# xu-ji/IIC

Measured on AMD Instinct MI355X. Metric: paired-images/sec, STL10 96x96 ClusterNet5g+IID_loss, higher is better.
Workload: dtype bf16; 1 GPU; STL10 96x96 ClusterNet5g IID+ (cluster_sobel.py train step), batch 660 pairs/GPU, 5 sub-heads, k=70, bf16 MFMA convs / fp32 stem+heads+loss, fused HIP Adam; global_batch_pairs=660, input=96x96x1 grey -> sobel 2ch, parallelism=dp1, streams=2, launch=hip-graph replay: 6 linear graph segments, the two views on two streams

## Files before the change

iic_amd/csrc/conv_igemm_bd.hip:

```cpp
#include "common.h"
#include "conv_tile.h"
#include "../../include/iic_hip.h"

__device__ __forceinline__ void bd_bload(u32x4& d, const unsigned char* p) {
  asm volatile("global_load_dwordx4 %0, %1, off" : "=v"(d) : "v"(p) : "memory");
}
template <int N>
__device__ __forceinline__ void bd_bwait(u32x4& d) {
  asm volatile("s_waitcnt vmcnt(%1)" : "+v"(d) : "i"(N) : "memory");
}

struct bd_blk {
  int bw, bh, nbx, nby;
  int PW, npix, mul;
};

#define BD_BM 256
#define BD_BN 128
#define BD_THREADS 256
#define BD_PROF_SLOTS 16
#ifndef BD_STORE_UB
#define BD_STORE_UB 8
#endif

// ... 293 lines not shown
      if (lane < 32) {
        const int col = wn * 64 + ns * 32 + lane;
        s_red[(wm * 2 + 0) * BNT + col] = s;
        s_red[(wm * 2 + 1) * BNT + col] = ss;
      }
    }
  }
  __syncthreads();
  if (stats && tid < BNT && !(ABL & 64)) {
    const int stripe = blockIdx.x % IIC_STAT_STRIPES;
    float a0 = 0.f, a1 = 0.f;
#pragma unroll
    for (int q = 0; q < NWM; ++q) {
      a0 += s_red[(q * 2 + 0) * BNT + tid];
      a1 += s_red[(q * 2 + 1) * BNT + tid];
    }
    iic_stat_add(stats, stripe, g.Cout, n0 + tid, 0, a0);
    iic_stat_add(stats, stripe, g.Cout, n0 + tid, 1, a1);
  }
#pragma unroll
  for (int ms = 0; ms < MS; ++ms)
#pragma unroll
    for (int ns = 0; ns < 2; ++ns)
#pragma unroll
      for (int r = 0; r < 16; ++r) {
        const int row = wm * WR + ms * 32 + mfma32_row(r, lane);
        const int col = wn * 64 + ns * 32 + l31;
        sC[row * CLD + col] = f32_to_bf16(acc[ms][ns][r]);
      }
  __syncthreads();
  if (PROF) t_stamp[4] = __builtin_readcyclecounter();
  TileRed tr;
  if (RED) tile_red_zero(tr);
  if (!(ABL & 32))
    igemm_store_tile<BNT, BM, BD_THREADS, 8, RED, (BM == 256 ? BD_STORE_UB : 4)>(sC, s_pout, out, res_grad, res_act, accumulate,
                                                                 g.Cout, n0, tid, red_y, red_coef, red_y2, &tr);
  if (RED)
    igemm_red_finish<BNT, BD_THREADS, RED>(tr, reinterpret_cast<float*>(smem_raw), red_stats, red_stats2,
                                             g.Cout, n0, tid);
  if (PROF && prof && tid == 0) {
    unsigned long long* q = prof + (long)blockIdx.x * BD_PROF_SLOTS;
    const unsigned long long t_end = __builtin_readcyclecounter();
    q[0] = t_stamp[0]; q[1] = t_stamp[1]; q[2] = t_stamp[2]; q[3] = t_stamp[3]; q[4] = t_stamp[4];
    q[5] = t_end; q[6] = t_bsum; q[7] = (unsigned long long)t_nb;
    q[8] = (unsigned long long)__builtin_amdgcn_s_getreg((32 - 1) << 11 | 0 << 6 | 4)
           | ((unsigned long long)__builtin_amdgcn_s_getreg((4 - 1) << 11 | 0 << 6 | 20) << 32);
    q[9] = (unsigned long long)tix;
    q[10] = __builtin_amdgcn_s_memrealtime();
  }
}

template <bool GATHER, int ABL, int MS, int RED, int WN = 2>
__global__ __launch_bounds__(BD_THREADS, ((MS == 4 || WN == 1) ? 2 : 3)) void conv_igemm_bd_kernel(
    const iic_conv_geom g, const bf16_t* __restrict__ in, const unsigned char* __restrict__ wfrag,
    bf16_t* __restrict__ out, float* __restrict__ stats, const bf16_t* __restrict__ res_grad,
    const bf16_t* __restrict__ res_act, int accumulate, int num_mtiles, int lds_a_bytes,
    const bf16_t* __restrict__ red_y, const float* __restrict__ red_coef,
    const bf16_t* __restrict__ red_y2, float* __restrict__ red_stats, float* __restrict__ red_stats2,
    unsigned long long* __restrict__ prof, const bd_blk B) {
  bd_tile<GATHER, ABL, MS, RED, WN>(g, in, wfrag, out, stats, res_grad, res_act, accumulate, lds_a_bytes, red_y,
                                    red_coef, red_y2, red_stats, red_stats2, prof, (int)blockIdx.x,
                                    num_mtiles * (g.Cout / (WN * 64)), B);
}

__global__ void weight_prep_frag_kernel(const float* __restrict__ w, bf16_t* __restrict__ o, int Co,
                                        int Ci, int T, int mode) {
  const int Nn = mode ? Ci : Co, Kk = mode ? Co : Ci;
  const int n32 = Nn >> 5, nchunks = Kk >> 6;
  const long total = (long)T * Co * Ci;
  for (long i = (long)blockIdx.x * blockDim.x + threadIdx.x; i < total;
       i += (long)gridDim.x * blockDim.x) {
    const int e = (int)(i & 7), lane = (int)((i >> 3) & 63), ks = (int)((i >> 9) & 3);
    long r = i >> 11;
    const int j = (int)(r % n32);
    r /= n32;
    const int kc = (int)(r % nchunks), t = (int)(r / nchunks);
    const int n = j * 32 + (lane & 31), k = kc * 64 + ks * 16 + (lane >> 5) * 8 + e;
    const int co = mode ? k : n, ci = mode ? n : k;
    o[i] = f32_to_bf16(w[((long)co * Ci + ci) * T + t]);
  }
}

int iic_p64_supported(const iic_conv_geom* g);
int iic_p64_launch(const iic_conv_geom* g, const void* in, const void* wfrag, void* out, float* stats,
                   const void* res_grad, const void* res_act, int accumulate, const void* red_y,
                   const float* red_coef, const void* red_y2, float* red_stats, float* red_stats2,
                   void* stream);
int iic_pw_supported(const iic_conv_geom* g);
int iic_pw_launch(const iic_conv_geom* g, const void* in, const void* wfrag, void* out, float* stats,
                  const void* res_grad, const void* res_act, int accumulate, const void* red_y,
                  const float* red_coef, const void* red_y2, float* red_stats, float* red_stats2, void* stream);
IIC_SWITCH(g_p64_enabled, 1, iic_debug_enable_p64)
IIC_SWITCH(g_p64_red, 0, iic_debug_p64_red)

extern "C" {

#ifdef IIC_DEBUG_HOOKS
static unsigned long long* g_bd_prof = nullptr;
IIC_HOOK void iic_debug_bd_prof(void* buf) { g_bd_prof = (unsigned long long*)buf; }
IIC_HOOK int iic_debug_bd_prof_slots(void) { return BD_PROF_SLOTS; }
#else
static constexpr unsigned long long* g_bd_prof = nullptr;
#endif

static long bd_lds_a(const iic_conv_geom* g, int ms, int wn = 2) {
  const long bm = ms * 32 * (4 / wn);
  const long npix = g->ntaps == 1 ? bm : (bm >= 192 ? g->NP256 : g->NP);
  long a = (npix * 128 + 1023) & ~1023L;
  long c = bm * (wn * 64 + 8) * 2;
  long m = a > c ? a : c;
  return (m + 15) & ~15L;
}

static long bd_key_bytes(const iic_conv_geom* g, int ms, int wn = 2) {
  const int jskip = (g->ntaps > 1 && g->sx == 1 && ((g->in_Wp - g->MX) & 1) == 0) ? g->in_Wp - g->MX : 0;
  return jskip != 0 ? (((long)(ms * 32 * (4 / wn) >= 192 ? g->NP256 : g->NP) + 15) & ~15L) : 0;
}
static long bd_lds_total(const iic_conv_geom* g, int ms, int wn = 2) {
  return bd_lds_a(g, ms, wn) + 2L * ms * 32 * (4 / wn) * 4 + 4L * BD_BN * 4 + bd_key_bytes(g, ms, wn);
}
IIC_SWITCH(g_bd_w1, 1, iic_debug_bd_w1)
static bool bd_w1_ok(const iic_conv_geom* g) {
  return g_bd_w1 && g->Cout % 64 == 0 && g->Cout % BD_BN != 0 && g->ntaps > 1 && g->NP256 > 0 &&
         bd_lds_total(g, 2, 1) <= 160 * 1024;
}
IIC_SWITCH(g_bd_ms, 0, iic_debug_bd_ms)
static int bd_pick_ms(const iic_conv_geom* g) {
  const bool ok4 = (g->ntaps == 1 || g->NP256 > 0) && bd_lds_total(g, 4) <= 160 * 1024;
  const bool ok2 = (g->ntaps == 1 || g->NP > 0) && bd_lds_total(g, 2) <= 160 * 1024;
  if (g_bd_ms == 4) return ok4 ? 4 : (ok2 ? 2 : 0);
  if (g_bd_ms == 2) return ok2 ? 2 : (ok4 ? 4 : 0);
  if (ok4 && ok2 && g->ntaps > 1) {
    const long M = igemm_rows_host(g);
    if (((M + 255) / 256) * (g->Cout / BD_BN) * 2 <= 512) return 2;
  }
  return ok4 ? 4 : (ok2 ? 2 : 0);
}

static int bd_block_config(const iic_conv_geom* g, bd_blk* B, int wn);
int iic_conv_igemm_frag_supported(const iic_conv_geom* g) {
  if (!g) return 0;
  if (g_p64_enabled && iic_p64_supported(g)) return 1;
  if (g->Cin % 64 != 0 || g->ntaps < 1 || g->ntaps > IIC_MAX_TAPS) return 0;
  bd_blk B;
  if (g->Cout % BD_BN != 0) return (bd_w1_ok(g) || (g->Cout % 64 == 0 && bd_block_config(g, &B, 1))) ? 1 : 0;
  return bd_pick_ms(g) != 0 || bd_block_config(g, &B, 2) != 0;
}

int iic_conv_igemm_frag_red(const iic_conv_geom* g, const void* in, const void* wfrag, void* out,
                            float* stats, const void* res_grad, const void* res_act, int accumulate,
                            const void* red_y, const float* red_coef, const void* red_y2,
                            float* red_stats, float* red_stats2, void* stream);

IIC_SWITCH(g_bd_blk, 1, iic_debug_bd_blk)
static int bd_block_config(const iic_conv_geom* g, bd_blk* B, int wn) {
  B->bw = 0;
  if (!g_bd_blk || g->ntaps < 2 || g->Cout % (wn * 64) != 0 || g->Cin % 64 != 0) return 0;
  if (g->sy != 1 || g->sx != 1 || g->ty != 1 || g->tx != 1 || g->MY < 32 || g->MX < 32 || g->NP256 <= 0) return 0;
  int mix = 0, miy = 0;
  for (int t = 0; t < g->ntaps; ++t) {
    const int iy = g->tap_off[t] / g->in_Wp, ix = g->tap_off[t] % g->in_Wp;
    if (ix > 8 || iy > 8) return 0;
    mix = ix > mix ? ix : mix;
    miy = iy > miy ? iy : miy;
  }
  if (mix & 1) return 0;
  double best = -1.0;
  int best_bw = 0;
  long best_tiles = 0;
  for (int bw = 8; bw <= 64 && bw <= g->MX; ++bw) {
    const int bh = BD_BM / bw;
    if (bh < 2 || bh > g->MY) continue;
    const long tiles = (long)((g->MX + bw - 1) / bw) * ((g->MY + bh - 1) / bh);
    const long npix = (long)(bw + mix) * (bh + miy);
    const long a = (npix * 128 + 1023) & ~1023L;
    const long c = (long)BD_BM * (wn * 64 + 8) * 2;
    const long tot = (a > c ? a : c) + 2L * BD_BM * 4 + 4L * BD_BN * 4 + ((npix + 15) & ~15L);
    if (tot > 80 * 1024 || npix >= 65536 / (bw + mix)) continue;
    const double cost = (double)tiles * (1.0 + 0.5 * (double)npix * 128.0 / 32768.0);
    if (best < 0 || cost < best) { best = cost; best_bw = bw; best_tiles = tiles; }
  }
  if (best < 0) return 0;
  const int bw = best_bw, bh = BD_BM / bw;
  if ((double)g->MY * g->MX < 0.88 * (double)BD_BM * (double)best_tiles) return 0;
  const int npix = (bw + mix) * (bh + miy);
  if (g_bd_blk != 2 && !(bd_lds_total(g, wn == 2 ? 4 : 2, wn) > 80 * 1024 || npix * 10 < g->NP256 * 7)) return 0;
  B->bw = bw; B->bh = bh;
  B->nbx = (g->MX + bw - 1) / bw; B->nby = (g->MY + bh - 1) / bh;
  B->PW = bw + mix; B->npix = npix; B->mul = (65536 + B->PW - 1) / B->PW;
  return 1;
}

int iic_conv_igemm_red_supported(const iic_conv_geom* g) {
  if (!g || !iic_conv_igemm_frag_supported(g)) return 0;
  if (g_p64_enabled && iic_p64_supported(g)) return g_p64_red;
  return g->ntaps > 1;
}

int iic_conv_igemm_frag(const iic_conv_geom* g, const void* in, const void* wfrag, void* out,
                        float* stats, const void* res_grad, const void* res_act, int accumulate,
                        void* stream) {
  return iic_conv_igemm_frag_red(g, in, wfrag, out, stats, res_grad, res_act, accumulate, nullptr, nullptr,
                                 nullptr, nullptr, nullptr, stream);
}

int iic_conv_igemm_frag_red(const iic_conv_geom* g, const void* in, const void* wfrag, void* out,
                            float* stats, const void* res_grad, const void* res_act, int accumulate,
                            const void* red_y, const float* red_coef, const void* red_y2,
                            float* red_stats, float* red_stats2, void* stream) {
  if (!g || !in || !wfrag || !out) return IIC_ERR_ARG;
  if ((red_y == nullptr) != (red_stats == nullptr) || (red_y2 == nullptr) != (red_stats2 == nullptr) ||
      (red_y2 && !red_y) || (red_coef && !red_y))
    return IIC_ERR_ARG;
  const int red = red_y ? (red_y2 ? 2 : 1) : 0;
  if (!(accumulate & IIC_ACC_PREMASK) && (res_grad == nullptr) != (res_act == nullptr)) return IIC_ERR_ARG;
  if (!iic_conv_igemm_frag_supported(g)) return IIC_ERR_UNSUPPORTED;
  if (g_p64_enabled && iic_p64_supported(g)) {
    if (red && !g_p64_red) return IIC_ERR_UNSUPPORTED;
    return iic_p64_launch(g, in, wfrag, out, stats, res_grad, res_act, accumulate, red_y, red_coef, red_y2,
                          red_stats, red_stats2, stream);
  }
  if (iic_debug_get_ablate() == 0 && g_bd_ms == 0 && iic_pw_supported(g))
    return iic_pw_launch(g, in, wfrag, out, stats, res_grad, res_act, accumulate, red_y, red_coef, red_y2, red_stats,
                         red_stats2, stream);
  const long M = igemm_rows_host(g);
  if (M <= 0) return IIC_ERR_ARG;
  if (M >= (1L << 31) || (long)g->N * g->in_Hp * g->in_Wp >= (1L << 31)) return IIC_ERR_UNSUPPORTED;
  if (g->Cout % BD_BN != 0) {
    bd_blk B1 = {0, 0, 0, 0, 0, 0, 0};
    const bool blocked1 = bd_block_config(g, &B1, 1) != 0;
    const int mt1 = blocked1 ? g->N * B1.nbx * B1.nby : (int)((M + 255) / 256);
    const int grid1 = mt1 * (g->Cout / 64);
    int la1 = (int)bd_lds_a(g, 2, 1);
    long lds1 = bd_lds_total(g, 2, 1);
    if (blocked1) {
      const long a = ((long)B1.npix * 128 + 1023) & ~1023L, c = (long)BD_BM * (64 + 8) * 2;
      la1 = (int)(((a > c ? a : c) + 15) & ~15L);
      lds1 = la1 + 2L * BD_BM * 4 + 4L * BD_BN * 4 + ((B1.npix + 15) & ~15L);
    }
    hipStream_t s1 = (hipStream_t)stream;
#define BD_LAUNCH_W1(RD_)                                                                              \
  do {                                                                                                 \
    static bool attr = false;                                                                          \
    if (!attr) {                                                                                       \
      (void)hipFuncSetAttribute(                                                                       \
          reinterpret_cast<const void*>(&conv_igemm_bd_kernel<false, 0, 2, RD_, 1>),          \
          hipFuncAttributeMaxDynamicSharedMemorySize, 160 * 1024);                                     \
      attr = true;                                                                                     \
    }                                                                                                  \
    hipLaunchKernelGGL((conv_igemm_bd_kernel<false, 0, 2, RD_, 1>), dim3(grid1),              \
                       dim3(BD_THREADS), lds1, s1, *g, (const bf16_t*)in, (const unsigned char*)wfrag, \
                       (bf16_t*)out, stats, (const bf16_t*)res_grad, (const bf16_t*)res_act,           \
                       accumulate, mt1, la1, (const bf16_t*)red_y, red_coef, (const bf16_t*)red_y2,    \
                       red_stats, red_stats2, (unsigned long long*)nullptr, B1);                       \
  } while (0)
    if (red == 0) BD_LAUNCH_W1(0); else if (red == 1) BD_LAUNCH_W1(1); else BD_LAUNCH_W1(2);
    return iic_launch_status();
  }
  bd_blk BB = {0, 0, 0, 0, 0, 0, 0};
  const bool blocked = iic_debug_get_ablate() == 0 && bd_block_config(g, &BB, 2) != 0;
  const int ms = blocked ? 4 : bd_pick_ms(g);
  if (ms == 0) return IIC_ERR_UNSUPPORTED;
  const int bm = ms * 64;
  const int mt = blocked ? g->N * BB.nbx * BB.nby : (int)((M + bm - 1) / bm);
  const int nt = g->Cout / BD_BN;
  const int grid = mt * nt;
  int la = (int)bd_lds_a(g, ms);
  long lds = bd_lds_total(g, ms);
  if (blocked) {
    const long a = ((long)BB.npix * 128 + 1023) & ~1023L, c = (long)BD_BM * (BD_BN + 8) * 2;
    la = (int)(((a > c ? a : c) + 15) & ~15L);
    lds = la + 2L * BD_BM * 4 + 4L * BD_BN * 4 + ((BB.npix + 15) & ~15L);
  }
  hipStream_t s = (hipStream_t)stream;
#define BD_LAUNCH4(GA_, AB_, MS_, RD_)                                                            \
  do {                                                                                           \
    static bool attr = false;                                                                    \
    if (!attr) {                                                                                 \
      (void)hipFuncSetAttribute(                                                                 \
          reinterpret_cast<const void*>(&conv_igemm_bd_kernel<GA_, AB_, MS_, RD_>),              \
          hipFuncAttributeMaxDynamicSharedMemorySize, 160 * 1024);                               \
      attr = true;                                                                               \
    }                                                                                            \
    hipLaunchKernelGGL((conv_igemm_bd_kernel<GA_, AB_, MS_, RD_>), dim3(grid),                   \
                       dim3(BD_THREADS), lds, s, *g, (const bf16_t*)in,                          \
                       (const unsigned char*)wfrag, (bf16_t*)out, stats, (const bf16_t*)res_grad, \
                       (const bf16_t*)res_act, accumulate, mt, la, (const bf16_t*)red_y,         \
                       red_coef, (const bf16_t*)red_y2, red_stats, red_stats2, g_bd_prof, BB);   \
  } while (0)
#define BD_LAUNCH3(GA_, AB_, MS_)                                                                 \
  do {                                                                                           \
    if ((AB_ != 0 && AB_ != 128 && AB_ != 256) || GA_ || red == 0) {                             \
      if (red != 0) return IIC_ERR_UNSUPPORTED;                                                  \
      BD_LAUNCH4(GA_, AB_, MS_, 0);                                                              \
    } else if (red == 1) BD_LAUNCH4(false, (AB_ == 128 || AB_ == 256 ? AB_ : 0), MS_, 1);        \
    else BD_LAUNCH4(false, (AB_ == 128 || AB_ == 256 ? AB_ : 0), MS_, 2);                        \
  } while (0)
#define BD_LAUNCH(GA_, AB_)                                                                       \
  do {                                                                                           \
    if (ms == 4) BD_LAUNCH3(GA_, AB_, 4); else BD_LAUNCH3(GA_, AB_, 2);                          \
  } while (0)
  if (g->ntaps == 1) BD_LAUNCH(true, 0);
  else switch (iic_debug_get_ablate()) {
// ... 86 lines not shown
```

iic_amd/csrc/conv_igemm_p64.hip:

```cpp
#include "common.h"
#include "conv_tile.h"
#include "../../include/iic_hip.h"

#define P64_BM 256
#define P64_BN 64
#define P64_THREADS 512
#define P64_NT 9
#define P64_CLD P64_BN
#define P64_SC_BYTES(BM_) ((BM_) * P64_CLD * 2)
#define P64_NTAB 4
#define P64_TAB_BYTES(BM_) (P64_NTAB * (BM_) * (4 + 2))

struct P64Walk {
  int n, y, x;
};
__device__ __forceinline__ void p64_walk_init(P64Walk& w, const iic_conv_geom& g, int m) {
  const int plane = g.MY * g.MX;
  w.n = m / plane;
  const int r = m - w.n * plane;
  w.y = r / g.MX;
  w.x = r - w.y * g.MX;
}
__device__ __forceinline__ void p64_walk_advance(P64Walk& w, const iic_conv_geom& g, int d_y, int d_x) {
  w.x += d_x;
  w.y += d_y;
  if (w.x >= g.MX) { w.x -= g.MX; ++w.y; }
  while (w.y >= g.MY) { w.y -= g.MY; ++w.n; }
}
__device__ __forceinline__ void p64_walk_pixels(const P64Walk& w, const iic_conv_geom& g, int& pin,
                                                int& pout) {
  const bool valid = w.n < g.N;
  const int n = valid ? w.n : g.N - 1, y = valid ? w.y : g.MY - 1, x = valid ? w.x : g.MX - 1;
  pin = (n * g.in_Hp + y * g.sy + g.oy) * g.in_Wp + x * g.sx + g.ox;
  pout = valid ? (n * g.out_Hp + y * g.ty + g.py) * g.out_Wp + x * g.tx + g.px : -1;
}

template <int ABL, int RED>
__global__ __launch_bounds__(512) void conv_igemm_p64_kernel(
    const iic_conv_geom g, const bf16_t* __restrict__ in, const unsigned char* __restrict__ wfrag,
    bf16_t* __restrict__ out, float* __restrict__ stats, const bf16_t* __restrict__ res_grad,
    const bf16_t* __restrict__ res_act, int accumulate, int num_tiles, int pb_bytes, int max_tap_off,
    const bf16_t* __restrict__ red_y, const float* __restrict__ red_coef,
    const bf16_t* __restrict__ red_y2, float* __restrict__ red_stats, float* __restrict__ red_stats2,
    unsigned long long* __restrict__ prof) {
  constexpr bool PROF = (ABL & 8) != 0;
  constexpr int NW = 8, BM = P64_BM;
  constexpr int NWM = BM / 64;
  constexpr int SC_BYTES = BM * P64_CLD * 2, TAB_ROWS = P64_NTAB * BM;
  unsigned long long ph[6] = {0, 0, 0, 0, 0, 0}, t_a = 0, t_b = 0, t_loop = 0;
  extern __shared__ __attribute__((aligned(16))) unsigned char smem_raw[];
  unsigned char* const sP0 = smem_raw;
  unsigned char* const sP1 = smem_raw + pb_bytes;
  bf16_t* const sC = reinterpret_cast<bf16_t*>(smem_raw + 2 * pb_bytes);
  int* const s_pout = reinterpret_cast<int*>(smem_raw + 2 * pb_bytes + SC_BYTES);
  unsigned short* const s_prow = reinterpret_cast<unsigned short*>(s_pout + TAB_ROWS);
  float* const s_red = reinterpret_cast<float*>(sC);

  constexpr int NTH = NW * 64;
  constexpr int NCO = 1;
  const int tid = threadIdx.x, lane = tid & 63;
  const int wave = __builtin_amdgcn_readfirstlane(tid >> 6);
  const int wm = wave >> 1, wn = wave & 1;
  const int l31 = lane & 31, g5 = lane >> 5;
  const int M = g.N * g.MY * g.MX;
  const int in_pixels = g.N * g.in_Hp * g.in_Wp;

  const int G = gridDim.x;
  const int wl = xcd_tile_index(blockIdx.x, G);
  const int t0 = (int)(((long)wl * num_tiles) / G), t1 = (int)(((long)(wl + 1) * num_tiles) / G);
  if (t0 >= t1) return;

  const int v_tapoff = g.tap_off[lane & (IIC_MAX_TAPS - 1)];
  const int d_y = BM / g.MX, d_x = BM - d_y * g.MX;

  P64Walk wr, w0, w255;
  p64_walk_init(wr, g, t0 * BM + (tid & (BM - 1)));
  p64_walk_init(w0, g, t0 * BM);
  p64_walk_init(w255, g, t0 * BM + BM - 1);
  int plo_q[3], nblk_q[3];
  auto tabulate = [&](int t) {
    int pin, pout, p0, p255, dummy;
    p64_walk_pixels(w0, g, p0, dummy);
    p64_walk_pixels(w255, g, p255, dummy);
    p0 = __builtin_amdgcn_readfirstlane(p0);
    p255 = __builtin_amdgcn_readfirstlane(p255);
    if (tid < BM) {
      p64_walk_pixels(wr, g, pin, pout);
      s_pout[(t & (P64_NTAB - 1)) * BM + tid] = pout;
      s_prow[(t & (P64_NTAB - 1)) * BM + tid] = (unsigned short)(pin - p0);
    }
    p64_walk_advance(wr, g, d_y, d_x);
    p64_walk_advance(w0, g, d_y, d_x);
    p64_walk_advance(w255, g, d_y, d_x);
    plo_q[0] = plo_q[1];
    nblk_q[0] = nblk_q[1];
    plo_q[1] = plo_q[2];
    nblk_q[1] = nblk_q[2];
    plo_q[2] = p0;
    nblk_q[2] = ((p255 + max_tap_off - p0 + 1) * 128 + 1023) >> 10;
  };
  auto dma_issue = [&](unsigned char* dst, int plo, int nblk) {
    for (int blk = wave; blk < nblk; blk += NW) {
      const int q = blk * 64 + lane;
      const int r = q >> 3;
      const int ls = (q & 7) ^ ((r >> 1) & 7);
      int p = plo + r;
      p = p < in_pixels ? p : in_pixels - 1;
      __builtin_amdgcn_global_load_lds(
          (const __attribute__((address_space(1))) void*)(in + ((long)p * 64 + ls * 8)),
          (__attribute__((address_space(3))) void*)(dst + blk * 1024), 16, 0, 0);
    }
  };

  tabulate(t0);
  tabulate(t0 + 1);
  dma_issue(sP0, plo_q[1], nblk_q[1]);
  u32x4 Bw[P64_NT][NCO][4];
#pragma unroll
  for (int tap = 0; tap < P64_NT; ++tap)
#pragma unroll
    for (int c = 0; c < NCO; ++c) {
      const unsigned char* p = wfrag + ((long)g.tap_w[tap] * 2 + wn + c) * 4096 + lane * 16;
#pragma unroll
      for (int ks = 0; ks < 4; ++ks) Bw[tap][c][ks] = *reinterpret_cast<const u32x4*>(p + ks * 1024);
    }
  f32x2 st_s[NCO], st_ss[NCO];
#pragma unroll
  for (int c = 0; c < NCO; ++c) {
    st_s[c] = f32x2{0.f, 0.f};
    st_ss[c] = f32x2{0.f, 0.f};
  }
  TileRed tr;
  if (RED) tile_red_zero(tr);

  if (PROF) t_loop = __builtin_readcyclecounter();
  for (int t = t0; t < t1; ++t) {
    const int par = (t - t0) & 1;
    unsigned char* const sP = par ? sP1 : sP0;
    if (PROF) t_a = __builtin_readcyclecounter();
    asm volatile("s_waitcnt vmcnt(0)" ::: "memory");
    __syncthreads();
    if (PROF) { t_b = __builtin_readcyclecounter(); ph[0] += t_b - t_a; t_a = t_b; }
    const bool spread = RED == 0 && !res_grad && !res_act && !accumulate;
    if (t > t0 && !(ABL & 2) && !spread)
      igemm_store_tile<P64_BN, BM, NTH, 0, RED, (RED ? 1 : 4)>(sC, s_pout + ((t - 1) & (P64_NTAB - 1)) * BM,
                                                            out, res_grad, res_act, accumulate, P64_BN, 0, tid,
                                                            red_y, red_coef, red_y2, &tr);
    if (PROF) { t_b = __builtin_readcyclecounter(); ph[1] += t_b - t_a; t_a = t_b; }
    if (t + 1 < t1 && !(ABL & 1)) dma_issue(par ? sP0 : sP1, plo_q[2], nblk_q[2]);
    tabulate(t + 2);
    if (PROF) { t_b = __builtin_readcyclecounter(); ph[2] += t_b - t_a; t_a = t_b; }
    int R0[2];
#pragma unroll
    for (int ms = 0; ms < 2; ++ms)
      R0[ms] = s_prow[(t & (P64_NTAB - 1)) * BM + wm * 64 + ms * 32 + l31];
    f32x16 acc[2][NCO];
    constexpr int NTAPS = (ABL & 4) ? 1 : P64_NT;
    auto load_a = [&](int tap, bf16x8 (&a)[2][4]) {
      const int toff = __builtin_amdgcn_readlane(v_tapoff, tap);
#pragma unroll
      for (int ms = 0; ms < 2; ++ms) {
        const int R = R0[ms] + toff;
        const int key = (R >> 1) & 7;
        const int base = R * 128 + (((g5 ^ key) & 1) << 4);
        const int kk = (key >> 1) << 5;
#pragma unroll
        for (int ks = 0; ks < 4; ++ks)
          a[ms][ks] = *reinterpret_cast<const bf16x8*>(sP + base + ((ks << 5) ^ kk));
      }
    };
#pragma unroll
    for (int tap = 0; tap < NTAPS; ++tap) {
      bf16x8 a[2][4];
      load_a(tap, a);
      if (spread && t > t0 && !(ABL & 2)) {
        constexpr int SIT = BM * 8 / NTH;
        constexpr int PER = (SIT + P64_NT - 2) / (P64_NT - 1);
#pragma unroll
        for (int q = 0; q < PER; ++q) {
          const int it = (tap - 1) * PER + q;
          if (tap >= 1 && it < SIT) {
            const int idx = tid + it * NTH;
            const int row = idx >> 3, ch = idx & 7;
            const int po = s_pout[((t - 1) & (P64_NTAB - 1)) * BM + row];
            if (po >= 0)
              *reinterpret_cast<uint4*>(out + (long)po * P64_BN + ch * 8) =
                  *reinterpret_cast<const uint4*>(sC + row * P64_CLD + ch * 8);
          }
        }
      }
#pragma unroll
      for (int ks = 0; ks < 4; ++ks)
#pragma unroll
        for (int c = 0; c < NCO; ++c) {
          const bf16x8 b = __builtin_bit_cast(bf16x8, Bw[tap][c][ks]);
          if (tap == 0 && ks == 0) {
            const f32x16 z = {0.f, 0.f, 0.f, 0.f, 0.f, 0.f, 0.f, 0.f, 0.f, 0.f, 0.f, 0.f, 0.f, 0.f, 0.f, 0.f};
            acc[0][c] = __builtin_amdgcn_mfma_f32_32x32x16_bf16(a[0][ks], b, z, 0, 0, 0);
            acc[1][c] = __builtin_amdgcn_mfma_f32_32x32x16_bf16(a[1][ks], b, z, 0, 0, 0);
          } else {
            acc[0][c] = __builtin_amdgcn_mfma_f32_32x32x16_bf16(a[0][ks], b, acc[0][c], 0, 0, 0);
            acc[1][c] = __builtin_amdgcn_mfma_f32_32x32x16_bf16(a[1][ks], b, acc[1][c], 0, 0, 0);
          }
        }
    }
    if (stats) {
      if ((t + 1) * BM > M) {
#pragma unroll
        for (int ms = 0; ms < 2; ++ms)
#pragma unroll
          for (int r = 0; r < 16; ++r)
            if (t * BM + wm * 64 + ms * 32 + mfma32_row(r, lane) >= M) {
#pragma unroll
              for (int c = 0; c < NCO; ++c) acc[ms][c][r] = 0.f;
            }
      }
#pragma unroll
      for (int c = 0; c < NCO; ++c)
#pragma unroll
        for (int ms = 0; ms < 2; ++ms)
#pragma unroll
          for (int r = 0; r < 16; r += 2) {
            const f32x2 v = {acc[ms][c][r], acc[ms][c][r + 1]};
            st_s[c] += v;
            st_ss[c] += v * v;
          }
    }
    if (PROF) { t_b = __builtin_readcyclecounter(); ph[3] += t_b - t_a; t_a = t_b; }
    asm volatile("s_waitcnt lgkmcnt(0)" ::: "memory");
    __builtin_amdgcn_s_barrier();
    if (PROF) { t_b = __builtin_readcyclecounter(); ph[4] += t_b - t_a; t_a = t_b; }
#pragma unroll
    for (int c = 0; c < NCO; ++c)
#pragma unroll
      for (int ms = 0; ms < 2; ++ms)
#pragma unroll
        for (int r = 0; r < 16; ++r)
          sC[(wm * 64 + ms * 32 + mfma32_row(r, lane)) * P64_CLD + (wn + c) * 32 + l31] = f32_to_bf16(acc[ms][c][r]);
    if (PROF) { t_b = __builtin_readcyclecounter(); ph[5] += t_b - t_a; }
  }
  if (PROF && prof && tid == 0) {
    unsigned long long* q = prof + (long)blockIdx.x * 8;
#pragma unroll
    for (int i = 0; i < 6; ++i) q[i] = ph[i];
    q[6] = (unsigned long long)(t1 - t0);
    q[7] = __builtin_readcyclecounter() - t_loop;
  }

  __syncthreads();
  if (!(ABL & 2))
    igemm_store_tile<P64_BN, BM, NTH, 0, RED, (RED ? 1 : 4)>(sC, s_pout + ((t1 - 1) & (P64_NTAB - 1)) * BM, out,
                                                          res_grad, res_act, accumulate, P64_BN, 0, tid,
                                                          red_y, red_coef, red_y2, &tr);
  if (RED)
    igemm_red_finish<P64_BN, NTH, RED>(tr, reinterpret_cast<float*>(sC), red_stats, red_stats2, P64_BN,
                                               0, tid);
  if (stats) {
    __syncthreads();
#pragma unroll
    for (int c = 0; c < NCO; ++c) {
      float s1 = st_s[c][0] + st_s[c][1], s2 = st_ss[c][0] + st_ss[c][1];
      s1 += __shfl_xor(s1, 32, 64);
      s2 += __shfl_xor(s2, 32, 64);
      if (lane < 32) {
        s_red[(wm * 2 + 0) * P64_BN + (wn + c) * 32 + lane] = s1;
        s_red[(wm * 2 + 1) * P64_BN + (wn + c) * 32 + lane] = s2;
      }
    }
    __syncthreads();
    if (tid < P64_BN) {
      float a0 = 0.f, a1 = 0.f;
#pragma unroll
      for (int q = 0; q < NWM; ++q) {
        a0 += s_red[(q * 2 + 0) * P64_BN + tid];
        a1 += s_red[(q * 2 + 1) * P64_BN + tid];
      }
      const int stripe = blockIdx.x % IIC_STAT_STRIPES;
      iic_stat_add(stats, stripe, P64_BN, tid, 0, a0);
      iic_stat_add(stats, stripe, P64_BN, tid, 1, a1);
    }
  }
}

#ifdef IIC_DEBUG_HOOKS
static unsigned long long* g_p64_prof = nullptr;
IIC_HOOK void iic_debug_p64_prof(void* buf) { g_p64_prof = (unsigned long long*)buf; }
#else
static constexpr unsigned long long* g_p64_prof = nullptr;
#endif
IIC_SWITCH(g_p64_grid, 0, iic_debug_p64_grid)

static int p64_num_cus() {
  if (g_p64_grid > 0) return g_p64_grid;
  static int n = 0;
  if (n == 0) {
    int dev = 0, v = 0;
    if (hipGetDevice(&dev) == hipSuccess &&
        hipDeviceGetAttribute(&v, hipDeviceAttributeMultiprocessorCount, dev) == hipSuccess && v > 0)
      n = v;
    else
      n = 256;
  }
  return n;
}

static long p64_pb_bytes(const iic_conv_geom* g, int bm = P64_BM) {
  return (((long)(bm == 128 ? g->NP : g->NP256) * 128) + 1023) & ~1023L;
}

int iic_p64_supported(const iic_conv_geom* g) {
  if (g->Cin != 64 || g->Cout != 64 || g->ntaps != P64_NT || g->NP256 <= 0 || g->NP256 > 65535) return 0;
  if (!igemm_dense_host(g)) return 0;
  return 2 * p64_pb_bytes(g) + P64_SC_BYTES(P64_BM) + P64_TAB_BYTES(P64_BM) <= 160 * 1024;
}

int iic_p64_launch(const iic_conv_geom* g, const void* in, const void* wfrag, void* out, float* stats,
                   const void* res_grad, const void* res_act, int accumulate, const void* red_y,
                   const float* red_coef, const void* red_y2, float* red_stats, float* red_stats2,
                   void* stream) {
  const int red = red_y ? (red_y2 ? 2 : 1) : 0;
  const long M = (long)g->N * g->MY * g->MX;
  if (M <= 0) return IIC_ERR_ARG;
  if (M >= (1L << 31) - P64_BM || (long)g->N * g->in_Hp * g->in_Wp >= (1L << 31)) return IIC_ERR_UNSUPPORTED;
  const int bm = P64_BM;
  const int nt = (int)((M + bm - 1) / bm);
  const int pb = (int)p64_pb_bytes(g, bm);
  const long lds = 2L * pb + P64_SC_BYTES(bm) + P64_TAB_BYTES(bm);
  int mto = 0;
  for (int i = 0; i < g->ntaps; ++i) mto = g->tap_off[i] > mto ? g->tap_off[i] : mto;
  const int ncu = p64_num_cus();
  const int grid = nt < ncu ? nt : ncu;
#define P64_LAUNCH2(AB_, RD_)                                                                          \
  do {                                                                                                 \
    static bool attr = false;                                                                          \
    if (!attr) {                                                                                       \
      (void)hipFuncSetAttribute(reinterpret_cast<const void*>(&conv_igemm_p64_kernel<AB_, RD_>),       \
                                hipFuncAttributeMaxDynamicSharedMemorySize, 160 * 1024);               \
      attr = true;                                                                                     \
    }                                                                                                  \
    hipLaunchKernelGGL((conv_igemm_p64_kernel<AB_, RD_>), dim3(grid), dim3(512), lds,                  \
                       (hipStream_t)stream, *g, (const bf16_t*)in, (const unsigned char*)wfrag,   \
                       (bf16_t*)out, stats, (const bf16_t*)res_grad, (const bf16_t*)res_act,      \
                       accumulate, nt, pb, mto, (const bf16_t*)red_y, red_coef,                   \
                       (const bf16_t*)red_y2, red_stats, red_stats2, g_p64_prof);                 \
  } while (0)
#define P64_LAUNCH(AB_) P64_LAUNCH2(AB_, 0)
  if (red == 1) { P64_LAUNCH2(0, 1); return iic_launch_status(); }
  if (red == 2) { P64_LAUNCH2(0, 2); return iic_launch_status(); }
  switch (iic_debug_get_ablate()) {
#ifdef IIC_BD_ABLATIONS
    case 1: P64_LAUNCH(1); break;
    case 2: P64_LAUNCH(2); break;
    case 3: P64_LAUNCH(3); break;
    case 4: P64_LAUNCH(4); break;
    case 7: P64_LAUNCH(7); break;
    case 8: P64_LAUNCH(8); break;
#endif
    default: P64_LAUNCH(0); break;
  }
  return iic_launch_status();
}
```

iic_amd/csrc/conv_tile.h:

```cpp
#pragma once
#include "common.h"
#include "../../include/iic_hip.h"

__device__ __forceinline__ void igemm_row_pixels(const iic_conv_geom& g, int m, int& pin, int& pout) {
  const int plane = g.MY * g.MX;
  const int mp = g.MP > 0 ? g.MP : plane;
  int n = m / mp;
  int r = m - n * mp;
  const bool valid = n < g.N && r < plane;
  if (n >= g.N) { n = g.N - 1; r = plane - 1; }
  r = r < plane ? r : plane - 1;
  const int y = r / g.MX, x = r - y * g.MX;
  pin = (n * g.in_Hp + y * g.sy + g.oy) * g.in_Wp + x * g.sx + g.ox;
  pout = valid ? (n * g.out_Hp + y * g.ty + g.py) * g.out_Wp + x * g.tx + g.px : -1;
}
__device__ __forceinline__ int igemm_rows(const iic_conv_geom& g) {
  return g.N * (g.MP > 0 ? g.MP : g.MY * g.MX);
}
__device__ __forceinline__ bool igemm_tile_has_invalid(const iic_conv_geom& g, int m0, int bm) {
  const int plane = g.MY * g.MX;
  if (m0 + bm > igemm_rows(g)) return true;
  return g.MP > 0 && g.MP != plane && (m0 % g.MP) + bm > plane;
}
static inline long igemm_rows_host(const iic_conv_geom* g) {
// ... 74 lines not shown
      const int idx = tid + (b0 + u) * NTHREADS;
      const int row = idx / CH;
      const int po = (idx < BM * CH) ? s_pout[row] : -1;
      o[u] = po < 0 ? -1 : (long)po * Cout + n0 + ch * 8;
      if (o[u] >= 0) {
        if (add_prev) pv[u] = *reinterpret_cast<const uint4*>(out + o[u]);
        if (res_grad) gv[u] = *reinterpret_cast<const uint4*>(res_grad + o[u]);
        if (res_act) av[u] = *reinterpret_cast<const uint4*>(res_act + o[u]);
        if (RED) yv[u] = *reinterpret_cast<const uint4*>(red_y + o[u]);
        if (RED == 2) zv[u] = *reinterpret_cast<const uint4*>(red_y2 + o[u]);
      }
    }
#pragma unroll
    for (int u = 0; u < U; ++u) {
      if (o[u] < 0) continue;
      const int row = (tid + (b0 + u) * NTHREADS) / CH;
      uint4 v = *reinterpret_cast<const uint4*>(sC + row * CLD + ch * 8);
      if (any_in) {
        uint32_t vv[4] = {v.x, v.y, v.z, v.w};
        float f[8];
#pragma unroll
        for (int i = 0; i < 4; ++i) { f[2 * i] = bf16lo(vv[i]); f[2 * i + 1] = bf16hi(vv[i]); }
        if (add_prev) {
          const uint32_t oo[4] = {pv[u].x, pv[u].y, pv[u].z, pv[u].w};
#pragma unroll
          for (int i = 0; i < 4; ++i) { f[2 * i] += bf16lo(oo[i]); f[2 * i + 1] += bf16hi(oo[i]); }
        }
        if (premask) {
          if (res_grad) {
            const uint32_t gg[4] = {gv[u].x, gv[u].y, gv[u].z, gv[u].w};
#pragma unroll
            for (int i = 0; i < 4; ++i) { f[2 * i] += bf16lo(gg[i]); f[2 * i + 1] += bf16hi(gg[i]); }
          }
          if (res_act) {
            const uint32_t aa[4] = {av[u].x, av[u].y, av[u].z, av[u].w};
#pragma unroll
            for (int i = 0; i < 4; ++i) {
              if (!(bf16lo(aa[i]) > 0.f)) f[2 * i] = 0.f;
              if (!(bf16hi(aa[i]) > 0.f)) f[2 * i + 1] = 0.f;
            }
          }
        } else if (res_grad) {
          const uint32_t gg[4] = {gv[u].x, gv[u].y, gv[u].z, gv[u].w};
          const uint32_t aa[4] = {av[u].x, av[u].y, av[u].z, av[u].w};
#pragma unroll
          for (int i = 0; i < 4; ++i) {
            if (bf16lo(aa[i]) > 0.f) f[2 * i] += bf16lo(gg[i]);
            if (bf16hi(aa[i]) > 0.f) f[2 * i + 1] += bf16hi(gg[i]);
          }
        }
        v = make_uint4(pack_bf16x2(f[0], f[1]), pack_bf16x2(f[2], f[3]), pack_bf16x2(f[4], f[5]),
                       pack_bf16x2(f[6], f[7]));
      }
      *reinterpret_cast<uint4*>(out + o[u]) = v;
      if (RED) {
        const uint32_t gq4[4] = {v.x, v.y, v.z, v.w};
        const uint32_t yy[4] = {yv[u].x, yv[u].y, yv[u].z, yv[u].w};
        float gq[8], yq[8];
#pragma unroll
        for (int i = 0; i < 4; ++i) {
          gq[2 * i] = bf16lo(gq4[i]); gq[2 * i + 1] = bf16hi(gq4[i]);
          yq[2 * i] = bf16lo(yy[i]); yq[2 * i + 1] = bf16hi(yy[i]);
        }
        if (red_coef) {
#pragma unroll
          for (int i = 0; i < 8; ++i)
            if (!(yq[i] * msc[RED ? i : 0] + msh[RED ? i : 0] > 0.f)) gq[i] = 0.f;
        }
#pragma unroll
        for (int i = 0; i < 8; ++i) { red->s[i] += gq[i]; red->sy[i] += gq[i] * yq[i]; }
        if (RED == 2) {
          const uint32_t zz[4] = {zv[u].x, zv[u].y, zv[u].z, zv[u].w};
#pragma unroll
          for (int i = 0; i < 4; ++i) {
            red->sy2[2 * i] += gq[2 * i] * bf16lo(zz[i]);
            red->sy2[2 * i + 1] += gq[2 * i + 1] * bf16hi(zz[i]);
          }
        }
      }
    }
  }
}

template <int BN, int NTHREADS, int RED>
__device__ __forceinline__ void igemm_red_finish(TileRed& r, float* scratch, float* red_stats,
                                                 float* red_stats2, int Cout, int n0, int tid) {
  constexpr int CH = BN / 8, NW = NTHREADS / 64;
  static_assert(64 % CH == 0, "channel chunks must divide the wave");
  const int lane = tid & 63, wave = tid >> 6, ch = tid % CH;
#pragma unroll
  for (int i = 0; i < 8; ++i) {
#pragma unroll
    for (int o = CH; o < 64; o <<= 1) {
      r.s[i] += __shfl_xor(r.s[i], o, 64);
      r.sy[i] += __shfl_xor(r.sy[i], o, 64);
      if (RED == 2) r.sy2[i] += __shfl_xor(r.sy2[i], o, 64);
    }
  }
  __syncthreads();
  if (lane < CH) {
#pragma unroll
    for (int i = 0; i < 8; ++i) {
      scratch[(wave * 3 + 0) * BN + ch * 8 + i] = r.s[i];
      scratch[(wave * 3 + 1) * BN + ch * 8 + i] = r.sy[i];
      if (RED == 2) scratch[(wave * 3 + 2) * BN + ch * 8 + i] = r.sy2[i];
    }
  }
  __syncthreads();
  if (tid < BN) {
    float a0 = 0.f, a1 = 0.f, a2 = 0.f;
    for (int w = 0; w < NW; ++w) {
      a0 += scratch[(w * 3 + 0) * BN + tid];
      a1 += scratch[(w * 3 + 1) * BN + tid];
      if (RED == 2) a2 += scratch[(w * 3 + 2) * BN + tid];
    }
    const int stripe = blockIdx.x % IIC_STAT_STRIPES;
    iic_stat_add(red_stats, stripe, Cout, n0 + tid, 0, a0);
    iic_stat_add(red_stats, stripe, Cout, n0 + tid, 1, a1);
    if (RED == 2) {
      iic_stat_add(red_stats2, stripe, Cout, n0 + tid, 0, a0);
      iic_stat_add(red_stats2, stripe, Cout, n0 + tid, 1, a2);
    }
  }
}
```

Before: 18750 paired-images/sec.

## Interleave p64 conv epilogue stores with MFMA tap loop for residual/reduction paths

Adds an EPI template variant of the p64 implicit-GEMM kernel. For tiles with residual, accumulate or reduction epilogues, it splits the previous tile's store into pieces and issues their global loads and stores between the taps of the current tile's MFMA loop, instead of running a separate store phase before the compute. This is meant to hide epilogue memory latency behind the matrix math. Reduction coefficients are staged in LDS, which needs extra LDS and adds new support checks. Fused stats with red are now rejected, and red==2 keeps the non-pipelined path.

```diff
diff --git a/iic_amd/csrc/conv_igemm_bd.hip b/iic_amd/csrc/conv_igemm_bd.hip
--- a/iic_amd/csrc/conv_igemm_bd.hip
+++ b/iic_amd/csrc/conv_igemm_bd.hip
@@ -399,10 +399,11 @@
 }
 
 int iic_p64_supported(const iic_conv_geom* g);
+int iic_p64_red_supported(const iic_conv_geom* g);
 int iic_p64_launch(const iic_conv_geom* g, const void* in, const void* wfrag, void* out, float* stats,
                    const void* res_grad, const void* res_act, int accumulate, const void* red_y,
                    const float* red_coef, const void* red_y2, float* red_stats, float* red_stats2,
-                   void* stream);
+                   int pipelined, void* stream);
 int iic_pw_supported(const iic_conv_geom* g);
 int iic_pw_launch(const iic_conv_geom* g, const void* in, const void* wfrag, void* out, float* stats,
                   const void* res_grad, const void* res_act, int accumulate, const void* red_y,
@@ -510,7 +511,7 @@
 
 int iic_conv_igemm_red_supported(const iic_conv_geom* g) {
   if (!g || !iic_conv_igemm_frag_supported(g)) return 0;
-  if (g_p64_enabled && iic_p64_supported(g)) return g_p64_red;
+  if (g_p64_enabled && iic_p64_supported(g)) return g_p64_red && iic_p64_red_supported(g);
   return g->ntaps > 1;
 }
 
@@ -533,9 +534,9 @@
   if (!(accumulate & IIC_ACC_PREMASK) && (res_grad == nullptr) != (res_act == nullptr)) return IIC_ERR_ARG;
   if (!iic_conv_igemm_frag_supported(g)) return IIC_ERR_UNSUPPORTED;
   if (g_p64_enabled && iic_p64_supported(g)) {
-    if (red && !g_p64_red) return IIC_ERR_UNSUPPORTED;
+    if (red && !(g_p64_red && iic_p64_red_supported(g))) return IIC_ERR_UNSUPPORTED;
     return iic_p64_launch(g, in, wfrag, out, stats, res_grad, res_act, accumulate, red_y, red_coef, red_y2,
-                          red_stats, red_stats2, stream);
+                          red_stats, red_stats2, g_p64_red, stream);
   }
   if (iic_debug_get_ablate() == 0 && g_bd_ms == 0 && iic_pw_supported(g))
     return iic_pw_launch(g, in, wfrag, out, stats, res_grad, res_act, accumulate, red_y, red_coef, red_y2, red_stats,
diff --git a/iic_amd/csrc/conv_igemm_p64.hip b/iic_amd/csrc/conv_igemm_p64.hip
--- a/iic_amd/csrc/conv_igemm_p64.hip
+++ b/iic_amd/csrc/conv_igemm_p64.hip
@@ -10,6 +10,7 @@
 #define P64_SC_BYTES(BM_) ((BM_) * P64_CLD * 2)
 #define P64_NTAB 4
 #define P64_TAB_BYTES(BM_) (P64_NTAB * (BM_) * (4 + 2))
+#define P64_COEF_BYTES (2 * P64_BN * 4)
 
 struct P64Walk {
   int n, y, x;
@@ -35,7 +36,7 @@
   pout = valid ? (n * g.out_Hp + y * g.ty + g.py) * g.out_Wp + x * g.tx + g.px : -1;
 }
 
-template <int ABL, int RED>
+template <int ABL, int RED, int EPI>
 __global__ __launch_bounds__(512) void conv_igemm_p64_kernel(
     const iic_conv_geom g, const bf16_t* __restrict__ in, const unsigned char* __restrict__ wfrag,
     bf16_t* __restrict__ out, float* __restrict__ stats, const bf16_t* __restrict__ res_grad,
@@ -55,6 +56,7 @@
   int* const s_pout = reinterpret_cast<int*>(smem_raw + 2 * pb_bytes + SC_BYTES);
   unsigned short* const s_prow = reinterpret_cast<unsigned short*>(s_pout + TAB_ROWS);
   float* const s_red = reinterpret_cast<float*>(sC);
+  float* const s_coef = reinterpret_cast<float*>(s_prow + TAB_ROWS);
 
   constexpr int NTH = NW * 64;
   constexpr int NCO = 1;
@@ -132,6 +134,8 @@
   }
   TileRed tr;
   if (RED) tile_red_zero(tr);
+  if (EPI && RED && red_coef && tid < 2 * P64_BN) s_coef[tid] = red_coef[tid];
+  const bool add_prev = accumulate & IIC_ACC_ADD, premask = accumulate & IIC_ACC_PREMASK;
 
   if (PROF) t_loop = __builtin_readcyclecounter();
   for (int t = t0; t < t1; ++t) {
@@ -142,7 +146,7 @@
     __syncthreads();
     if (PROF) { t_b = __builtin_readcyclecounter(); ph[0] += t_b - t_a; t_a = t_b; }
     const bool spread = RED == 0 && !res_grad && !res_act && !accumulate;
-    if (t > t0 && !(ABL & 2) && !spread)
+    if (!EPI && t > t0 && !(ABL & 2) && !spread)
       igemm_store_tile<P64_BN, BM, NTH, 0, RED, (RED ? 1 : 4)>(sC, s_pout + ((t - 1) & (P64_NTAB - 1)) * BM,
                                                             out, res_grad, res_act, accumulate, P64_BN, 0, tid,
                                                             red_y, red_coef, red_y2, &tr);
@@ -169,6 +173,51 @@
           a[ms][ks] = *reinterpret_cast<const bf16x8*>(sP + base + ((ks << 5) ^ kk));
       }
     };
+    if constexpr (EPI != 0) {
+      TilePiece<RED> pc;
+      int pc_po = -1;
+      const int ch = tid & 7;
+      const bool pipe = t > t0 && !(ABL & 2);
+      const int* const po_tab = s_pout + ((t - 1) & (P64_NTAB - 1)) * BM;
+#pragma unroll
+      for (int tap = 0; tap < NTAPS; ++tap) {
+        if (pipe && (tap & 1) == 0) {
+          if (tap >= 2 && pc_po >= 0) {
+            pc.o = (long)pc_po * P64_BN + ch * 8;
+            const int row = (tap / 2 - 1) * (NTH / 8) + (tid >> 3);
+            const uint4 v = *reinterpret_cast<const uint4*>(sC + row * P64_CLD + ch * 8);
+            igemm_piece_finish<RED>(pc, v, out, res_grad != nullptr, res_act != nullptr, add_prev, premask,
+                                    red_coef != nullptr, s_coef + ch * 8, s_coef + P64_BN + ch * 8, &tr);
+          }
+          if (tap < 8) {
+            pc_po = po_tab[(tap / 2) * (NTH / 8) + (tid >> 3)];
+            pc.o = (long)pc_po * P64_BN + ch * 8;
+            if (pc_po >= 0) igemm_piece_load<RED>(pc, out, res_grad, res_act, add_prev, red_y, red_y2);
+          }
+        }
+        const int toff = __builtin_amdgcn_readlane(v_tapoff, tap);
+#pragma unroll
+        for (int ms = 0; ms < 2; ++ms) {
+          const int R = R0[ms] + toff;
+          const int key = (R >> 1) & 7;
+          const int base = R * 128 + (((g5 ^ key) & 1) << 4);
+          const int kk = (key >> 1) << 5;
+          bf16x8 a[4];
+#pragma unroll
+          for (int ks = 0; ks < 4; ++ks) a[ks] = *reinterpret_cast<const bf16x8*>(sP + base + ((ks << 5) ^ kk));
+#pragma unroll
+          for (int ks = 0; ks < 4; ++ks) {
+            const bf16x8 b = __builtin_bit_cast(bf16x8, Bw[tap][0][ks]);
+            if (tap == 0 && ks == 0) {
+              const f32x16 z = {0.f, 0.f, 0.f, 0.f, 0.f, 0.f, 0.f, 0.f, 0.f, 0.f, 0.f, 0.f, 0.f, 0.f, 0.f, 0.f};
+              acc[ms][0] = __builtin_amdgcn_mfma_f32_32x32x16_bf16(a[ks], b, z, 0, 0, 0);
+            } else {
+              acc[ms][0] = __builtin_amdgcn_mfma_f32_32x32x16_bf16(a[ks], b, acc[ms][0], 0, 0, 0);
+            }
+          }
+        }
+      }
+    } else {
 #pragma unroll
     for (int tap = 0; tap < NTAPS; ++tap) {
       bf16x8 a[2][4];
@@ -204,7 +253,8 @@
           }
         }
     }
-    if (stats) {
+    }
+    if (RED == 0 && stats) {
       if ((t + 1) * BM > M) {
 #pragma unroll
         for (int ms = 0; ms < 2; ++ms)
@@ -255,7 +305,7 @@
   if (RED)
     igemm_red_finish<P64_BN, NTH, RED>(tr, reinterpret_cast<float*>(sC), red_stats, red_stats2, P64_BN,
                                                0, tid);
-  if (stats) {
+  if (RED == 0 && stats) {
     __syncthreads();
 #pragma unroll
     for (int c = 0; c < NCO; ++c) {
@@ -313,11 +363,15 @@
   if (!igemm_dense_host(g)) return 0;
   return 2 * p64_pb_bytes(g) + P64_SC_BYTES(P64_BM) + P64_TAB_BYTES(P64_BM) <= 160 * 1024;
 }
+int iic_p64_red_supported(const iic_conv_geom* g) {
+  return iic_p64_supported(g) &&
+         2 * p64_pb_bytes(g) + P64_SC_BYTES(P64_BM) + P64_TAB_BYTES(P64_BM) + P64_COEF_BYTES <= 160 * 1024;
+}
 
 int iic_p64_launch(const iic_conv_geom* g, const void* in, const void* wfrag, void* out, float* stats,
                    const void* res_grad, const void* res_act, int accumulate, const void* red_y,
                    const float* red_coef, const void* red_y2, float* red_stats, float* red_stats2,
-                   void* stream) {
+                   int pipelined, void* stream) {
   const int red = red_y ? (red_y2 ? 2 : 1) : 0;
   const long M = (long)g->N * g->MY * g->MX;
   if (M <= 0) return IIC_ERR_ARG;
@@ -325,38 +379,41 @@
   const int bm = P64_BM;
   const int nt = (int)((M + bm - 1) / bm);
   const int pb = (int)p64_pb_bytes(g, bm);
-  const long lds = 2L * pb + P64_SC_BYTES(bm) + P64_TAB_BYTES(bm);
+  const bool epi = pipelined && (red || res_grad || res_act || accumulate);
+  const long lds = 2L * pb + P64_SC_BYTES(bm) + P64_TAB_BYTES(bm) + (red ? P64_COEF_BYTES : 0);
+  if (lds > 160 * 1024) return IIC_ERR_UNSUPPORTED;
   int mto = 0;
   for (int i = 0; i < g->ntaps; ++i) mto = g->tap_off[i] > mto ? g->tap_off[i] : mto;
   const int ncu = p64_num_cus();
   const int grid = nt < ncu ? nt : ncu;
-#define P64_LAUNCH2(AB_, RD_)                                                                          \
+#define P64_LAUNCH(AB_, RD_, EP_)                                                                      \
   do {                                                                                                 \
     static bool attr = false;                                                                          \
     if (!attr) {                                                                                       \
-      (void)hipFuncSetAttribute(reinterpret_cast<const void*>(&conv_igemm_p64_kernel<AB_, RD_>),       \
+      (void)hipFuncSetAttribute(reinterpret_cast<const void*>(&conv_igemm_p64_kernel<AB_, RD_, EP_>),  \
                                 hipFuncAttributeMaxDynamicSharedMemorySize, 160 * 1024);               \
       attr = true;                                                                                     \
     }                                                                                                  \
-    hipLaunchKernelGGL((conv_igemm_p64_kernel<AB_, RD_>), dim3(grid), dim3(512), lds,                  \
-                       (hipStream_t)stream, *g, (const bf16_t*)in, (const unsigned char*)wfrag,   \
-                       (bf16_t*)out, stats, (const bf16_t*)res_grad, (const bf16_t*)res_act,      \
-                       accumulate, nt, pb, mto, (const bf16_t*)red_y, red_coef,                   \
-                       (const bf16_t*)red_y2, red_stats, red_stats2, g_p64_prof);                 \
+    hipLaunchKernelGGL((conv_igemm_p64_kernel<AB_, RD_, EP_>), dim3(grid), dim3(512), lds,             \
+                       (hipStream_t)stream, *g, (const bf16_t*)in, (const unsigned char*)wfrag,        \
+                       (bf16_t*)out, stats, (const bf16_t*)res_grad, (const bf16_t*)res_act,           \
+                       accumulate, nt, pb, mto, (const bf16_t*)red_y, red_coef,                        \
+                       (const bf16_t*)red_y2, red_stats, red_stats2, g_p64_prof);                      \
   } while (0)
-#define P64_LAUNCH(AB_) P64_LAUNCH2(AB_, 0)
-  if (red == 1) { P64_LAUNCH2(0, 1); return iic_launch_status(); }
-  if (red == 2) { P64_LAUNCH2(0, 2); return iic_launch_status(); }
+  if (red && stats) return IIC_ERR_UNSUPPORTED;
+  if (red && !pipelined) return IIC_ERR_UNSUPPORTED;
+  if (red == 1) { P64_LAUNCH(0, 1, 1); return iic_launch_status(); }
+  if (red == 2) { P64_LAUNCH(0, 2, 0); return iic_launch_status(); }
   switch (iic_debug_get_ablate()) {
 #ifdef IIC_BD_ABLATIONS
-    case 1: P64_LAUNCH(1); break;
-    case 2: P64_LAUNCH(2); break;
-    case 3: P64_LAUNCH(3); break;
-    case 4: P64_LAUNCH(4); break;
-    case 7: P64_LAUNCH(7); break;
-    case 8: P64_LAUNCH(8); break;
+    case 1: P64_LAUNCH(1, 0, 0); break;
+    case 2: P64_LAUNCH(2, 0, 0); break;
+    case 3: P64_LAUNCH(3, 0, 0); break;
+    case 4: P64_LAUNCH(4, 0, 0); break;
+    case 7: P64_LAUNCH(7, 0, 0); break;
+    case 8: if (epi) P64_LAUNCH(8, 0, 1); else P64_LAUNCH(8, 0, 0); break;
 #endif
-    default: P64_LAUNCH(0); break;
+    default: if (epi) P64_LAUNCH(0, 0, 1); else P64_LAUNCH(0, 0, 0); break;
   }
   return iic_launch_status();
 }
diff --git a/iic_amd/csrc/conv_tile.h b/iic_amd/csrc/conv_tile.h
--- a/iic_amd/csrc/conv_tile.h
+++ b/iic_amd/csrc/conv_tile.h
@@ -180,6 +180,94 @@
   }
 }
 
+template <int RED>
+struct TilePiece {
+  long o;
+  uint4 pv, gv, av, yv, zv;
+};
+
+template <int RED>
+__device__ __forceinline__ void igemm_piece_load(TilePiece<RED>& p, const bf16_t* __restrict__ out,
+                                                 const bf16_t* __restrict__ res_grad,
+                                                 const bf16_t* __restrict__ res_act, bool add_prev,
+                                                 const bf16_t* __restrict__ red_y,
+                                                 const bf16_t* __restrict__ red_y2) {
+  if (add_prev) p.pv = *reinterpret_cast<const uint4*>(out + p.o);
+  if (res_grad) p.gv = *reinterpret_cast<const uint4*>(res_grad + p.o);
+  if (res_act) p.av = *reinterpret_cast<const uint4*>(res_act + p.o);
+  if (RED) p.yv = *reinterpret_cast<const uint4*>(red_y + p.o);
+  if (RED == 2) p.zv = *reinterpret_cast<const uint4*>(red_y2 + p.o);
+}
+
+template <int RED>
+__device__ __forceinline__ void igemm_piece_finish(const TilePiece<RED>& p, uint4 v, bf16_t* __restrict__ out,
+                                                   bool has_grad, bool has_act, bool add_prev, bool premask,
+                                                   bool has_coef, const float* msc, const float* msh,
+                                                   TileRed* red) {
+  if (add_prev || has_grad || has_act) {
+    uint32_t vv[4] = {v.x, v.y, v.z, v.w};
+    float f[8];
+#pragma unroll
+    for (int i = 0; i < 4; ++i) { f[2 * i] = bf16lo(vv[i]); f[2 * i + 1] = bf16hi(vv[i]); }
+    if (add_prev) {
+      const uint32_t oo[4] = {p.pv.x, p.pv.y, p.pv.z, p.pv.w};
+#pragma unroll
+      for (int i = 0; i < 4; ++i) { f[2 * i] += bf16lo(oo[i]); f[2 * i + 1] += bf16hi(oo[i]); }
+    }
+    if (premask) {
+      if (has_grad) {
+        const uint32_t gg[4] = {p.gv.x, p.gv.y, p.gv.z, p.gv.w};
+#pragma unroll
+        for (int i = 0; i < 4; ++i) { f[2 * i] += bf16lo(gg[i]); f[2 * i + 1] += bf16hi(gg[i]); }
+      }
+      if (has_act) {
+        const uint32_t aa[4] = {p.av.x, p.av.y, p.av.z, p.av.w};
+#pragma unroll
+        for (int i = 0; i < 4; ++i) {
+          if (!(bf16lo(aa[i]) > 0.f)) f[2 * i] = 0.f;
+          if (!(bf16hi(aa[i]) > 0.f)) f[2 * i + 1] = 0.f;
+        }
+      }
+    } else if (has_grad) {
+      const uint32_t gg[4] = {p.gv.x, p.gv.y, p.gv.z, p.gv.w};
+      const uint32_t aa[4] = {p.av.x, p.av.y, p.av.z, p.av.w};
+#pragma unroll
+      for (int i = 0; i < 4; ++i) {
+        if (bf16lo(aa[i]) > 0.f) f[2 * i] += bf16lo(gg[i]);
+        if (bf16hi(aa[i]) > 0.f) f[2 * i + 1] += bf16hi(gg[i]);
+      }
+    }
+    v = make_uint4(pack_bf16x2(f[0], f[1]), pack_bf16x2(f[2], f[3]), pack_bf16x2(f[4], f[5]),
+                   pack_bf16x2(f[6], f[7]));
+  }
+  *reinterpret_cast<uint4*>(out + p.o) = v;
+  if (RED) {
+    const uint32_t gq4[4] = {v.x, v.y, v.z, v.w};
+    const uint32_t yy[4] = {p.yv.x, p.yv.y, p.yv.z, p.yv.w};
+    float gq[8], yq[8];
+#pragma unroll
+    for (int i = 0; i < 4; ++i) {
+      gq[2 * i] = bf16lo(gq4[i]); gq[2 * i + 1] = bf16hi(gq4[i]);
+      yq[2 * i] = bf16lo(yy[i]); yq[2 * i + 1] = bf16hi(yy[i]);
+    }
+    if (has_coef) {
+#pragma unroll
+      for (int i = 0; i < 8; ++i)
+        if (!(yq[i] * msc[i] + msh[i] > 0.f)) gq[i] = 0.f;
+    }
+#pragma unroll
+    for (int i = 0; i < 8; ++i) { red->s[i] += gq[i]; red->sy[i] += gq[i] * yq[i]; }
+    if (RED == 2) {
+      const uint32_t zz[4] = {p.zv.x, p.zv.y, p.zv.z, p.zv.w};
+#pragma unroll
+      for (int i = 0; i < 4; ++i) {
+        red->sy2[2 * i] += gq[2 * i] * bf16lo(zz[i]);
+        red->sy2[2 * i + 1] += gq[2 * i + 1] * bf16hi(zz[i]);
+      }
+    }
+  }
+}
+
 template <int BN, int NTHREADS, int RED>
 __device__ __forceinline__ void igemm_red_finish(TileRed& r, float* scratch, float* red_stats,
                                                  float* red_stats2, int Cout, int n0, int tid) {
```

New measurement: 18750 paired-images/sec (median of 2 runs). No clear change (-0.0%).
